# AgoraIO-Community/Solo

Hardware: AMD Instinct MI355X
Metric: 40 ms frames/sec (encode+decode) per GPU; concurrent real-time WB streams @1/2/4/8 MI355X (higher is better)
Workload: dtype int32 fixed point (int16 PCM, Q-format arithmetic, bit-exact); 1 GPU; BASELINE configs[2]: 4096 synthetic 16 kHz WB streams, full encode -> two-description bitstream -...; streams_per_gpu=4096, input_workers=16, launch=single process

## Files before the change

solo_amd/csrc/solo_common.h:

```cpp
#pragma once
#include "solo_wave.h"

#if defined(__HIPCC__)
#define SOLO_TAB static __device__ const
#else
#define SOLO_TAB static const
#endif
#include "solo_tables.inc"

#ifndef SX_FS_KHZ
#define SX_FS_KHZ 8
#endif
#if SX_FS_KHZ == 8
#define SX_LPC 10
#define SX_NLSF_STAGES 6
#define SX_NLSF_CB0_NVEC_TOTAL 120
#define SX_NLSF_CB1_NVEC_TOTAL 72
#define SX_NLSF_CB_MAXVEC 120
#define SX_MSVQ_ROW 16
#define SX_N_NLSF_CB0_CDF 126
#define SX_N_NLSF_CB1_CDF 78
#define SX_N_PITCH_LAG_CDF 130
#define SX_N_PITCH_CONTOUR_CDF 12
#define SX_PITCH_CB_N 11
// ... 356 lines not shown
        const u32 tot = sx_uadd_sat(nrg, pre);
        const unsigned long long cross = __builtin_amdgcn_ballot_w64(tot >= 0x80000000u);
        if (!cross) { nrg = (u32)__builtin_amdgcn_readlane((i32)tot, 63); break; }
        const int Lc = __builtin_ctzll(cross);
        u32 base = nrg;
        if (Lc > 0) base += (u32)__builtin_amdgcn_readlane((i32)pre, Lc - 1);
        bool found = false;
#pragma unroll
        for (int j = 0; j < MAXC; j++) {
            const int m = Lc * C + j;
            const u32 pj = (u32)__builtin_amdgcn_readlane((i32)P[j], Lc);
            if (!found && j < C && m >= cur) {
                base += pj >> shft;
                if (base >= 0x80000000u) { found = true; cur = m + 1; }
            }
        }
        nrg = base >> 2;
        shft += 2;
    }
    if (tail) nrg += (u32)sx_smulbb(x[len - 1], x[len - 1]) >> shft;
    if (nrg & 0xC0000000u) { nrg >>= 2; shft += 2; }
    *shift = shft;
    *energy = (i32)nrg;
}
template <int MAXC = 4>
SX_FN void sx_sum_sqr_shift_wv(i32* energy, i32* shift, const i16* x, int len, int odd_start) { sx_sum_sqr_shift_wv_inl<MAXC>(energy, shift, x, len, odd_start); }
#else
template <int MAXC = 4>
SX_HD void sx_sum_sqr_shift_wv(i32* energy, i32* shift, const i16* x, int len, int odd_start) { sx_sum_sqr_shift(energy, shift, x, len, odd_start); }
template <int MAXC>
SX_HD void sx_sum_sqr_shift_wv_inl(i32* energy, i32* shift, const i16* x, int len, int odd_start) { sx_sum_sqr_shift(energy, shift, x, len, odd_start); }
#endif

SX_HD void sx_lpc_analysis_filter_zero_state(const i16* in, const i16* B, i16* out, int len, int order) {
    SX_PAR(k, len) {
        i32 acc = 0;
        for (int j = 0; j < order; j++) {
            int t = k - 1 - j;
            if (t >= 0) acc = sx_smlabb(acc, in[t], B[j]);
        }
        i32 o = sx_sub_sat32(sx_shl((i32)in[k], 12), acc);
        out[k] = (i16)sx_sat16(sx_rshift_round(o, 12));
    }
}

SX_HD i32 sx_sigm_Q15(i32 in_Q5) {
    if (in_Q5 < 0) {
        in_Q5 = -in_Q5;
        if (in_Q5 >= 6 * 32) return 0;
        int ind = in_Q5 >> 5;
        return T_sigm_neg_Q15[ind] - sx_smulbb(T_sigm_slope_Q10[ind], in_Q5 & 0x1F);
    }
    if (in_Q5 >= 6 * 32) return 32767;
    int ind = in_Q5 >> 5;
    return T_sigm_pos_Q15[ind] + sx_smulbb(T_sigm_slope_Q10[ind], in_Q5 & 0x1F);
}

#ifdef SX_LANE_STREAM
#define SX_ROWB(v, jj) __shfl((v), (SX_LANE & 48) | (jj), 64)
#define SX_ROWG(v, idx) __shfl((v), (SX_LANE & 48) | ((idx) & 15), 64)
#define SX_ROW_NEXT(v) SX_DPP_((v), 0x101)

SX_HD void sx_row_nlsf_weights_laroia(i32* pW_Q6, const i32* pNLSF_Q15, int D, bool row_active) {
    const int k = SX_LANE & 15;
    i32 inv = 0;
    if (row_active && k <= D) {
        const i32 lo = k > 0 ? pNLSF_Q15[k - 1] : 0, hi = k < D ? pNLSF_Q15[k] : (1 << 15);
        inv = (1 << 21) / sx_max(hi - lo, 3);
    }
    const i32 nx = SX_ROW_NEXT(inv);
    if (row_active && k < D) pW_Q6[k] = sx_min(inv + nx, 32767);
}

template <int ORDER>
SX_HD i32 sx_row_inv_pred_gain_Q16_n(i32 a, bool* unstable) {
// ... 86 lines not shown
```

solo_amd/csrc/solo_enc.h:

```cpp
#pragma once
#include <stddef.h>
#include "solo_enc_analysis.h"
#if defined(SOLO_HOST_EMU)
#include "solo_enc_nsq_row.h"
#endif
#include "solo_cdf.h"

struct SxFrameIdx {
    i32 sigtype, QuantOffsetType;
    i32 GainsIndices[SX_NB_SUBFR], DeltaGainsIndices;
    i32 NLSFIndices[SX_NLSF_STAGES], NLSFInterpCoef_Q2;
    i32 lagIndex, contourIndex, PERIndex, LTPIndex[SX_NB_SUBFR], LTP_scaleIndex;
    i32 Seed, vadFlag;
    i32 inDTX, pad_;
};

#define SX_RC_PW_SIGNS (SX_FRAME + 2 * (SX_FRAME / 16) + 8 - ((SX_FRAME + 2 * (SX_FRAME / 16)) & 7))
#define SX_RC_PW_ROW (SX_RC_PW_SIGNS + SX_FRAME / 8 + (((SX_RC_PW_SIGNS + SX_FRAME / 8) / 4) & 1 ? 0 : 4))
static_assert(((SX_RC_PW_ROW / 4) & 1) == 1 && SX_RC_PW_ROW % 4 == 0, "odd dword rows");
#define SX_RC_BUF_STRIDE (SX_MAX_ARITHM_BYTES + 16)
struct SxRcInfo { i32 nBytes, error; };

struct SxCodeWork {
#if SX_NLANES == 1
    u8 buf[2][SX_RC_BUF_STRIDE];
    alignas(4) u8 pulses[SX_RC_PW_ROW];
    SxCdf cdf;
#else
    i32 unused_;
#endif
};

struct SxFrontWork {
    i16 x_buf[SX_XBUF];
    i16 res_pitch[2 * SX_FRAME + SX_LA_PITCH];
    i16 Wsig[SX_PITCH_LPC_WIN];
    union {
        SxPitchWork pitch;
        SxShapeWork shape;
        SxPredWork pred;
        SxPrefWork pref;
    } u;
};

struct SxHbWork {
    i16 x_hb_buf[SX_HB_XBUF];
    i16 lpc_in[4 * (10 * SX_FS_KHZ + SX_HB_LPC)];
    i16 exc[2 * SX_FRAME];
    i32 NLSF_Q15[SX_MAX_LPC];
    i32 weight[SX_MAX_LPC];
    i16 A_Q12[SX_MAX_LPC];
    i32 ws[SX_NLSF2A_WS];
    SxLpcWork lpc;
};

#define SX_HB_Q (SX_FS_KHZ == 8 ? 10 : 8)
struct SxEncWork {
    SxEncState st;
    SxEncCtrl ctrl;
    i16 xfw[SX_FRAME];
    u8 hb_bytes[8 * SX_HB_Q];
    union {
        i16 qmf_tl[63 + SX_PACKET];
        SxFrontWork front;
#if defined(SOLO_HOST_EMU)
        SxRowWork nsq;
#endif
        SxCodeWork code;
        SxHbWork hb;
    } u;
};

SX_HD void sx_enc_split(SxRangeEnc* rc, int p_child1, int p, const u16* shell_table, const SxCdf* cdf) {
    if (p > 0) sx_rc_enc(rc, p_child1, &shell_table[cdf->shell_offsets[p]]);
}

// ... 529 lines not shown
```

solo_amd/csrc/solo_enc_analysis.h:

```cpp
#pragma once
#include "solo_enc_front.h"
#include "solo_dec.h"

SX_FN void sx_warped_autocorr(i32* corr, i32* scale, const i16* input, i32 warping_Q16, int length) {
    const int order = SX_SHAPE_ORDER;
    i32 state[SX_SHAPE_ORDER + 1];
    i64 corr_QC[SX_SHAPE_ORDER + 1];
    for (int i = 0; i <= order; i++) { state[i] = 0; corr_QC[i] = 0; }
    for (int n = 0; n < length; n++) {
        i32 tmp1 = sx_shl((i32)input[n], 14), tmp2;
        for (int i = 0; i < order; i += 2) {
            tmp2 = sx_smlawb(state[i], state[i + 1] - tmp1, warping_Q16);
            state[i] = tmp1;
            corr_QC[i] += sx_smull(tmp1, state[0]) >> 18;
            tmp1 = sx_smlawb(state[i + 1], state[i + 2] - tmp2, warping_Q16);
            state[i + 1] = tmp2;
            corr_QC[i + 1] += sx_smull(tmp2, state[0]) >> 18;
        }
        state[order] = tmp1;
        corr_QC[order] += sx_smull(tmp1, state[0]) >> 18;
    }
    int lsh = sx_clz64(corr_QC[0]) - 35;
    lsh = sx_limit(lsh, -12 - 10, 30 - 10);
    *scale = -(10 + lsh);
// ... 1149 lines not shown
SX_FN void sx_burg_modified(i32* res_nrg, i32* res_nrg_Q, i32* A_Q16, const i16* x, int subfr_length, int nb_subfr, i32 WhiteNoiseFrac_Q32,
                            int D, SxBurgWork* bw) {
    SX_IN_LDS(x); SX_IN_LDS(bw); SX_IN_LDS(A_Q16);
    const int QA = 25, MAX_RSHIFTS = 32 - 25, MIN_RSHIFTS = -16;
    subfr_length = SX_UNI(subfr_length); nb_subfr = SX_UNI(nb_subfr); D = SX_UNI(D); WhiteNoiseFrac_Q32 = SX_UNI(WhiteNoiseFrac_Q32);
    const int L = subfr_length;
    i32 C0, rshifts;
    SX_T_BEGIN
    constexpr int PAIRS_PER_LANE = SITE == 2 ? (4 * (10 * SX_FS_KHZ + SX_HB_LPC) / 2 + 63) / 64 : (4 * (SX_SUBFR + SX_MAX_LPC) / 2 + 63) / 64;
    sx_sum_sqr_shift_wv_inl<PAIRS_PER_LANE>(&C0, &rshifts, x, nb_subfr * subfr_length, 0);
    C0 = SX_UNI(C0); rshifts = SX_UNI(rshifts);
    SX_T(23)
    if (rshifts > MAX_RSHIFTS) {
        C0 = sx_shl(C0, rshifts - MAX_RSHIFTS);
        rshifts = MAX_RSHIFTS;
    } else {
        int lz = sx_clz32(C0) - 1;
        int rshifts_extra = 2 - lz;
        if (rshifts_extra > 0) {
            rshifts_extra = sx_min(rshifts_extra, MAX_RSHIFTS - rshifts);
            C0 = C0 >> rshifts_extra;
        } else {
            rshifts_extra = sx_max(rshifts_extra, MIN_RSHIFTS - rshifts);
            C0 = sx_shl(C0, -rshifts_extra);
        }
        rshifts += rshifts_extra;
    }
    C0 = SX_UNI(C0); rshifts = SX_UNI(rshifts);
#if defined(SX_BURG_COUNT) && SX_NLANES == 1
    SX_BURG_COUNTED(SITE, rshifts > -2 ? 0 : 1);
    if (SITE == 1 && sx_burg_last_regime == (rshifts > 0)) SX_BURG_COUNTED(SITE, 3);
    if (SITE == 0) sx_burg_last_regime = rshifts > 0;
#endif
    SX_PAR(sn, nb_subfr * 16) {
        const int s = sn >> 4, n = (sn & 15) + 1;
        i32 v = 0;
        if (n <= D) {
            const i16* xs = x + s * L;
            if (rshifts > 0) {
                i64 acc = 0;
                for (int i = 0; i < L - n; i++) acc += (i64)((i32)xs[i] * (i32)xs[i + n]);
                v = (i32)(acc >> rshifts);
            } else {
                i32 acc = 0;
                for (int i = 0; i < L - n; i++) acc = sx_smlabb(acc, xs[i], xs[i + n]);
                v = sx_shl(acc, -rshifts);
            }
        }
        bw->p1[sn] = v;
    }
    wv_sync();
    SX_PAR(k, SX_MAX_LPC) {
        i32 v = 0;
        for (int s = 0; s < nb_subfr; s++) v = sx_add(v, bw->p1[s * 16 + k]);
        bw->Cf[k] = v;
        bw->Cl[k] = v;
        bw->Af[k] = 0;
    }
    SX_T(24)
    const i32 CA0 = sx_add(sx_add(C0, sx_smmul(WhiteNoiseFrac_Q32, C0)), 1);
    bw->CAf[0] = CA0;
    bw->CAb[0] = CA0;
    wv_sync();
#if defined(__HIP_DEVICE_COMPILE__) && SX_NLANES == 64 && SX_FS_KHZ == 8
    i32 nrg, tmp1;
    {
        const int row = SX_LANE >> 4, k = SX_LANE & 15, rowbase = SX_LANE & 48;
        const bool live = row < nb_subfr;
        const i16* xr = x + (live ? row : 0) * L;
        const bool upper = row >= 2;
        i32 Af_k = 0, P_k = upper ? (k == 0 ? CA0 : 0) : bw->Cf[k], Q_k = P_k;
        i32 ef = live ? (i32)xr[k] : 0, eb = live ? (i32)xr[L - 1 - k] : 0, fr = 0, bk = 0;
#define SX_ROW_DOWN(v) __builtin_amdgcn_update_dpp(0, (v), 0x101, 0xF, 0xF, true)
#define SX_ROW_UP_IN(in, v) __builtin_amdgcn_update_dpp((in), (v), 0x111, 0xF, 0xF, false)
#define SX_ROW_BCAST0(v) __builtin_amdgcn_update_dpp(0, (v), 0x150, 0xF, 0xF, true)
// ... 426 lines not shown
                    i++;
                    if (i > 30) {
                        NLSF[0] = (1 << 15) / (d + 1);
                        for (k = 1; k < d; k++) NLSF[k] = sx_smulbb(k + 1, NLSF[0]);
                        wv_sync();
                        return;
                    }
                    wv_sync();
                    sx_bwexpander_32(a_Q16, d, 65536 - sx_smulbb(10 + i, i));
                    retry = true;
                    break;
                }
            }
        }
#endif
        wv_sync();
        if (!retry) return;
    }
}

SX_FN1 void sx_find_LPC(i32* NLSF_Q15, i32* interpIndex, const i32* prev_NLSFq_Q15, int useInterp, int order, const i16* x,
                       int subfr_length, i16* LPC_res, SxLpcWork* lw) {
    SX_IN_LDS(NLSF_Q15); SX_IN_LDS(interpIndex); SX_IN_LDS(prev_NLSFq_Q15); SX_IN_LDS(x); SX_IN_LDS(LPC_res); SX_IN_LDS(lw);
    i32* a_Q16 = lw->a_Q16;
    i32* a_tmp_Q16 = lw->a_tmp_Q16;
    i32 res_nrg, res_tmp_nrg, res_nrg_Q, res_tmp_nrg_Q;
    order = SX_LPC; subfr_length = SX_SUBFR + SX_LPC;
    *interpIndex = 4;
    sx_burg_modified(&res_nrg, &res_nrg_Q, a_Q16, x, subfr_length, 4, K_FIND_LPC_COND_FAC_Q32, order, &lw->burg);
    sx_bwexpander_32(a_Q16, order, K_FIND_LPC_CHIRP_Q16);
    wv_sync();
    SX_T_BEGIN
    if (useInterp == 1) {
        sx_burg_modified<1>(&res_tmp_nrg, &res_tmp_nrg_Q, a_tmp_Q16, x + 2 * subfr_length, subfr_length, 2, K_FIND_LPC_COND_FAC_Q32, order, &lw->burg);
        sx_bwexpander_32(a_tmp_Q16, order, K_FIND_LPC_CHIRP_Q16);
        wv_sync();
        SX_T(22)
        int shift = res_tmp_nrg_Q - res_nrg_Q;
        if (shift >= 0) {
            if (shift < 32) res_nrg = res_nrg - (res_tmp_nrg >> shift);
        } else {
            res_nrg = (res_nrg >> (-shift)) - res_tmp_nrg;
            res_nrg_Q = res_tmp_nrg_Q;
        }
        sx_a2nlsf<1>(NLSF_Q15, a_tmp_Q16, order, lw->P, lw->Q, &lw->u.grid);
        wv_sync();
        SX_T(21)
#if defined(SX_LANE_STREAM) && defined(SX_HAVE_ROW_NLSF2A)
        bool all_ok;
        {
            const int k = SX_LANE >> 4, i = SX_LANE & 15;
            if (i < SX_LPC) lw->u.it.NLSF0[k][i] = prev_NLSFq_Q15[i] + (sx_mul(NLSF_Q15[i] - prev_NLSFq_Q15[i], k) >> 2);
            wv_sync();
            all_ok = __builtin_amdgcn_ballot_w64(!sx_row_nlsf2a_stable(lw->u.it.a_Q12[k], lw->u.it.NLSF0[k])) == 0;
            wv_sync();
        }
        if (!all_ok)
#endif
        {
            SX_S(55)
            SX_PAR(k, 4) {
                for (int i = 0; i < order; i++) lw->u.it.NLSF0[k][i] = prev_NLSFq_Q15[i] + (sx_mul(NLSF_Q15[i] - prev_NLSFq_Q15[i], k) >> 2);
                sx_nlsf2a_stable_ws(lw->u.it.a_Q12[k], lw->u.it.NLSF0[k], order, lw->u.it.ws[k]);
            }
            wv_sync();
        }
        SX_S(53)
        {
            const int len = 2 * (SX_SUBFR + SX_LPC);
            SX_PAR(t, 4 * len) {
                const int k = t / len, n = t - k * len;
                const i16* B = lw->u.it.a_Q12[k];
                i32 acc = 0;
                for (int j = 0; j < order; j++) {
                    const int u = n - 1 - j;
                    if (u >= 0) acc = sx_smlabb(acc, x[u], B[j]);
                }
                const i32 o = sx_sub_sat32(sx_shl((i32)x[n], 12), acc);
                lw->u.it.res[k][n] = (i16)sx_sat16(sx_rshift_round(o, 12));
            }
        }
        wv_sync();
        SX_S(54)
        SX_PAR(kh, 8) {
            const int k = kh >> 1, h = kh & 1;
            i32 e, sh;
            sx_sum_sqr_shift_n<SX_SUBFR>(&e, &sh, lw->u.it.res[k] + order + h * subfr_length, 0);
            lw->u.it.nrg[k][h] = e;
            lw->u.it.rsh[k][h] = sh;
        }
        wv_sync();
        for (int k = 3; k >= 0; k--) {
            i32 res_nrg0 = lw->u.it.nrg[k][0], res_nrg1 = lw->u.it.nrg[k][1], res_nrg_interp, res_nrg_interp_Q;
            const i32 rshift0 = lw->u.it.rsh[k][0], rshift1 = lw->u.it.rsh[k][1];
            shift = rshift0 - rshift1;
            if (shift >= 0) {
                res_nrg1 = res_nrg1 >> shift;
                res_nrg_interp_Q = -rshift0;
            } else {
                res_nrg0 = res_nrg0 >> (-shift);
                res_nrg_interp_Q = -rshift1;
            }
            res_nrg_interp = sx_add(res_nrg0, res_nrg1);
            shift = res_nrg_interp_Q - res_nrg_Q;
            int isInterpLower;
            if (shift >= 0) {
                isInterpLower = (res_nrg_interp >> shift) < res_nrg;
            } else {
                isInterpLower = (-shift < 32) ? (res_nrg_interp < (res_nrg >> (-shift))) : 0;
            }
            if (isInterpLower) {
                res_nrg = res_nrg_interp;
// ... 344 lines not shown
    if (doInterpolate) {
        SX_PAR(i, SX_LPC) w->NLSF0[i] = st->prev_NLSFq_Q15[i] + (sx_mul(pNLSF_Q15[i] - st->prev_NLSFq_Q15[i], interp_Q2) >> 2);
        wv_sync();
    }
#if defined(SX_LANE_STREAM) && defined(SX_HAVE_ROW_NLSF2A)
    bool both_ok;
    {
        const int v = (SX_LANE >> 4) & 1;
        bool ok = true;
        if (doInterpolate) ok = sx_row_nlsf2a_stable(c->PredCoef_Q12[v], v ? pNLSF_Q15 : w->NLSF0);
        else ok = sx_row_nlsf2a_stable(c->PredCoef_Q12[1], pNLSF_Q15);
        both_ok = __builtin_amdgcn_ballot_w64(!ok) == 0;
        wv_sync();
    }
    if (!both_ok)
#endif
    {
        SX_S(56)
        SX_PAR(v, 2) {
            if (v == 1 || doInterpolate) sx_nlsf2a_stable_ws(c->PredCoef_Q12[v], v ? pNLSF_Q15 : w->NLSF0, SX_LPC, w->ws[v]);
        }
        wv_sync();
    }
    if (!doInterpolate) {
        SX_PAR(i, SX_LPC) c->PredCoef_Q12[0][i] = c->PredCoef_Q12[1][i];
        wv_sync();
    }
}

SX_FN1 void sx_residual_energy(i32* nrgs, i32* nrgsQ, const i16* x, i16 a_Q12[2][SX_MAX_LPC], const i32* gains, i16* LPC_res) {
    const int offset = SX_LPC + SX_SUBFR;
    const i16* x_ptr = x;
    for (int i = 0; i < 2; i++) {
        sx_lpc_analysis_filter_zero_state(x_ptr, a_Q12[i], LPC_res, 2 * offset, SX_LPC);
        wv_sync();
        for (int j = 0; j < 2; j++) {
            i32 rshift;
            static_assert(SX_SUBFR <= 128, "one pair of samples per lane");
            sx_sum_sqr_shift_wv_inl<1>(&nrgs[i * 2 + j], &rshift, LPC_res + SX_LPC + j * offset, SX_SUBFR, 0);
            nrgsQ[i * 2 + j] = -rshift;
        }
        x_ptr += 2 * offset;
        wv_sync();
    }
    for (int i = 0; i < 4; i++) {
        int lz1 = sx_clz32(nrgs[i]) - 1, lz2 = sx_clz32(gains[i]) - 1;
        i32 tmp32 = sx_shl(gains[i], lz2);
        tmp32 = sx_smmul(tmp32, tmp32);
        nrgs[i] = sx_smmul(tmp32, sx_shl(nrgs[i], lz1));
        nrgsQ[i] += lz1 + 2 * lz2 - 32 - 32;
    }
}

struct SxPredWork {
    i32 WLTP[4 * 25];
    i16 LPC_in_pre[4 * (SX_SUBFR + SX_LPC)];
    i16 LPC_res[2 * (SX_SUBFR + SX_LPC)];
    i32 NLSF_Q15[SX_MAX_LPC];
    i32 invGains_Q16[SX_NB_SUBFR], local_gains[SX_NB_SUBFR], Wght_Q15[SX_NB_SUBFR];
    union {
        SxLtpWork ltp;
        struct { i32 rd[3 * 4 * 40]; i32 best[3 * 4 * 2]; } vq;
        SxLpcWork lpc;
        SxMsvqWork msvq;
    } u;
};

// ... 134 lines not shown
```

solo_amd/csrc/solo_enc_front.h:

```cpp
#pragma once
#include "solo_enc_state.h"

SX_FN1 void sx_qmf_decomp(SxEncHist* hist, const i16* pcm, i16* tl, i16* lo, i16* hi, int n = SX_PACKET) {
    SX_IN_LDS(tl);
    n = SX_UNI(n);
    SX_PAR(i, 63) tl[i] = hist->qmf_hist[i];
    SX_PAR(i, n) tl[63 + i] = (i16)(pcm[i] >> 1);
    wv_sync();
    SX_PAR(k, n >> 1) {
        i32 y1 = 0, y2 = 0;
        const i16* xa = tl + 2 * k;
        const i16* xb = tl + 63 + 2 * k;
        for (int j = 0; j < 32; j++) {
            i32 a = T_qmf_taps[63 - j];
            i32 p = xa[j], q = xb[-j];
            y1 = sx_add(y1, sx_mul(a, (i32)(i16)(p + q)));
            i32 d = sx_mul(a, (i32)(i16)(p - q));
            y2 = (j & 1) ? sx_add(y2, d) : sx_sub(y2, d);
        }
        lo[k] = (i16)sx_saturate(sx_pshr32(y1, 15), 32767);
        hi[k] = (i16)sx_saturate(sx_pshr32(y2, 15), 32767);
    }
    wv_sync();
    SX_PAR(i, 63) hist->qmf_hist[i] = tl[n + i];
// ... 528 lines not shown
    const int min_lag_4 = 8, max_lag_4 = 72, min_lag_8 = 16, max_lag_8 = 144, sf8 = 40;
    constexpr int dn_C = (int)((offsetof(SxPitchWork, C) - offsetof(SxPitchWork, tmp32)) / sizeof(i32));
    static_assert(offsetof(SxPitchWork, tmp32) % 16 == 0 && offsetof(SxPitchWork, C) % 16 == 0 && sizeof(w->tmp32) >= 160 * sizeof(i32) &&
                  sizeof(w->C) >= 160 * sizeof(i32), "all-pass chains of the 8 -> 4 kHz decimator");
#if SX_FS_KHZ == 8
    SX_PAR(i, 320) w->sig8[i] = signal[i];
    wv_sync();
#else
    static_assert(offsetof(SxPitchWork, sig16) + sizeof(w->sig16) - offsetof(SxPitchWork, C) >= 640 * sizeof(i32), "all-pass chains of the 16 -> 8 kHz decimator");
    sx_down2_zero_state<640>(w->sig8, signal, w->tmp32 + dn_C, 320);
#endif
    sx_down2_zero_state<320>(w->sig4, w->sig8, w->tmp32, dn_C);
    SX_PAR(i, 4 * 221) (&w->C[0][0])[i] = 0;
#if SX_NLANES == 1
    for (int i = 159; i > 0; i--) w->sig4[i] = (i16)sx_sat16((i32)w->sig4[i] + (i32)w->sig4[i - 1]);
#else
    {
        i32 a[3];
#pragma unroll
        for (int j = 0; j < 3; j++) {
            const int i = SX_LANE + 64 * j;
            a[j] = (i > 0 && i < 160) ? sx_sat16((i32)w->sig4[i] + (i32)w->sig4[i - 1]) : 0;
        }
        wv_sync();
#pragma unroll
        for (int j = 0; j < 3; j++) { const int i = SX_LANE + 64 * j; if (i > 0 && i < 160) w->sig4[i] = (i16)a[j]; }
        wv_sync();
    }
#endif
    i32 shift = sx_pitch_find_scaling(w->sig4, 160, sx_max(sf8, 80));
    if (shift > 0) {
        SX_PAR(i, 160) w->sig4[i] = (i16)(w->sig4[i] >> shift);
        wv_sync();
    }
    SX_S(34)
    {
        i32 E8k[2], N8k[2];
        for (int k = 0; k < 2; k++) {
            const i16* b = &w->sig4[80 + k * sf8] - min_lag_4;
            i32 E8 = 0;
            SX_PAR(n, sf8) E8 = sx_smlabb(E8, b[n], b[n]);
            E8 = wv_sum(E8);
            E8k[k] = E8;
            N8k[k] = sx_add_sat32(E8, sx_smulbb(sf8, 4000));
        }
        const int nlag = max_lag_4 - min_lag_4 + 1;
        SX_PAR(t, 2 * nlag) {
            const int k = t / nlag, d = min_lag_4 + (t - k * nlag);
            const i16* target = &w->sig4[80 + k * sf8];
            const i16* b = target - d;
            i32 cc = 0, E = 0;
            for (int n = 0; n < sf8; n++) { cc = sx_smlabb(cc, target[n], b[n]); E = sx_smlabb(E, b[n], b[n]); }
            i32 normalizer = sx_add(k ? N8k[1] : N8k[0], sx_sub(E, k ? E8k[1] : E8k[0]));
            i32 tq = cc / (sx_sqrt_approx(normalizer) + 1);
            w->C[k][d] = (i16)sx_sat16(tq);
        }
        wv_sync();
    }
    SX_PAR(i, max_lag_4 + 1) {
        if (i >= min_lag_4) {
            i32 sum = ((i32)w->C[0][i] + (i32)w->C[1][i]) >> 1;
            sum = sx_smlawb(sum, sum, sx_shl(-i, 4));
            w->tmp32[i] = sum;
        }
    }
    wv_sync();
    int length_d_srch = 4 + 2 * 2;
    const int L = max_lag_4 - min_lag_4 + 1;
#if SX_NLANES == 64 && defined(__HIP_DEVICE_COMPILE__)
    {
        static_assert(72 - 8 + 1 == 65, "one element more than lanes");
        const int i = SX_LANE;
        const i32 v = (i16)w->tmp32[min_lag_4 + i], vl = (i16)w->tmp32[min_lag_4 + L - 1];
        int rank = 0;
        for (int j = 0; j < L; j++) {
            i32 u = (i16)w->tmp32[min_lag_4 + j];
            rank += (u > v || (u == v && j < i)) ? 1 : 0;
        }
        const int rank_last = __builtin_popcountll(__builtin_amdgcn_ballot_w64(v >= vl));
        wv_sync();
        if (rank < length_d_srch) { w->C[0][min_lag_4 + rank] = (i16)v; w->d_srch[rank] = i; }
        if (SX_LANE == 0 && rank_last < length_d_srch) { w->C[0][min_lag_4 + rank_last] = (i16)vl; w->d_srch[rank_last] = L - 1; }
    }
#else
    SX_PAR(i, L) {
// ... 64 lines not shown
        for (int j = 0; j < 3; j++) { const int i = SX_LANE + 64 * j; if (i >= min_lag_8 && i <= max_lag_8 + 3) w->d_comp[i] = (i16)m[j]; }
        wv_sync();
        int n_srch = 0;
#pragma unroll
        for (int j = 0; j < 3; j++) {
            const int i = SX_LANE + 64 * j;
            const bool pr = i >= min_lag_8 && i <= max_lag_8 && w->d_comp[i + 1] > 0;
            const unsigned long long bal = __builtin_amdgcn_ballot_w64(pr);
            if (pr) w->d_srch[n_srch + __builtin_popcountll(bal & below)] = i;
            n_srch += __builtin_popcountll(bal);
        }
        length_d_srch = n_srch;
#pragma unroll
        for (int j = 0; j < 3; j++) {
            const int i = SX_LANE + 64 * j;
            m[j] = (i >= min_lag_8 && i <= max_lag_8 + 3) ? (i32)w->d_comp[i] + w->d_comp[i - 1] + w->d_comp[i - 2] + w->d_comp[i - 3] : 0;
        }
        wv_sync();
#pragma unroll
        for (int j = 0; j < 3; j++) {
            const int i = SX_LANE + 64 * j;
            const bool pr = i >= min_lag_8 && i <= max_lag_8 + 3 && m[j] > 0;
            const unsigned long long bal = __builtin_amdgcn_ballot_w64(pr);
            if (pr) w->d_comp[length_d_comp + __builtin_popcountll(bal & below)] = (i16)(i - 2);
            length_d_comp += __builtin_popcountll(bal);
        }
        wv_sync();
    }
#endif
    SX_S(35)
    shift = sx_pitch_find_scaling(w->sig8, 320, sf8);
    if (shift > 0) {
        SX_PAR(i, 320) w->sig8[i] = (i16)(w->sig8[i] >> shift);
    }
    SX_PAR(i, 4 * 221) (&w->C[0][0])[i] = 0;
    wv_sync();
    SX_PAR(t, 4 * length_d_comp) {
        int k = t / length_d_comp, j = t - k * length_d_comp;
        const i16* tp = &w->sig8[160 + k * sf8];
        int d = w->d_comp[j];
        const i16* bp = tp - d;
        i32 cross = 0, eb = 0, et = 0;
        for (int n = 0; n < sf8; n++) {
            cross = sx_smlabb(cross, tp[n], bp[n]);
            eb = sx_smlabb(eb, bp[n], bp[n]);
            et = sx_smlabb(et, tp[n], tp[n]);
        }
        i32 r = 0;
        if (cross > 0) {
            i32 en = sx_max(et, eb);
            i32 lz = sx_clz32(cross);
            i32 lshift = sx_limit(lz - 1, 0, 15);
            i32 t32 = sx_shl(cross, lshift) / ((en >> (15 - lshift)) + 1);
            t32 = sx_smulwb(cross, t32);
            t32 = sx_add_sat32(t32, t32);
            lz = sx_clz32(t32);
            lshift = sx_limit(lz - 1, 0, 15);
            en = sx_min(et, eb);
            r = sx_shl(t32, lshift) / ((en >> (15 - lshift)) + 1);
        }
        w->C[k][d] = (i16)r;
    }
    wv_sync();
    i32 CCmax = SX_I32_MIN, CCmax_b = SX_I32_MIN;
    int CBimax = 0, lag = -1;
#if SX_FS_KHZ == 16
    if (prevLag > 0) prevLag = prevLag >> 1;
#endif
    i32 prevLag_log2_Q7 = prevLag > 0 ? sx_lin2log(prevLag) : 0;
    i32 corr_thres_Q15 = sx_smulbb(search_thres2_Q15, search_thres2_Q15) >> 13;
    SX_S(36)
    const int nb_cbks = SX_FS_KHZ == 8 ? 11 : 3;
#if SX_NLANES == 1
    for (int k = 0; k < length_d_srch; k++) {
        int d = w->d_srch[k];
        i32 CCmax_new = SX_I32_MIN;
        int CBimax_new = 0;
        for (int j = 0; j < nb_cbks; j++) {
            i32 cc = 0;
            for (int i = 0; i < 4; i++) cc += (i32)w->C[i][d + T_pitch_cb_stage2[i * 11 + j]];
// ... 19 lines not shown
    {
        i32 best_b = SX_I32_MIN, best_k = SX_I32_MAX, my_cc = 0, my_cb = 0;
        const int k = SX_LANE;
        if (k < length_d_srch) {
            const int d = w->d_srch[k];
            i32 CCmax_new = SX_I32_MIN;
            int CBimax_new = 0;
            for (int j = 0; j < nb_cbks; j++) {
                i32 cc = 0;
                for (int i = 0; i < 4; i++) cc += (i32)w->C[i][d + T_pitch_cb_stage2[i * 11 + j]];
                if (cc > CCmax_new) { CCmax_new = cc; CBimax_new = j; }
            }
            i32 lag_log2_Q7 = sx_lin2log(d);
            i32 CCmax_new_b = CCmax_new - (sx_smulbb(4 * 6554, lag_log2_Q7) >> 7);
            if (prevLag > 0) {
                i32 dl = lag_log2_Q7 - prevLag_log2_Q7;
                dl = sx_smulbb(dl, dl) >> 7;
                i32 bias = sx_smulbb(4 * 6554, *LTPCorr_Q15) >> 15;
                bias = sx_mul(bias, dl) / (dl + (1 << 6));
                CCmax_new_b -= bias;
            }
            if (CCmax_new_b > SX_I32_MIN && CCmax_new > corr_thres_Q15 && T_pitch_cb_stage2[CBimax_new] <= min_lag_8) {
                best_b = CCmax_new_b; best_k = k; my_cc = CCmax_new; my_cb = CBimax_new;
            }
        }
        wv_argmax(&best_b, &best_k);
        if (best_k != SX_I32_MAX && best_b > SX_I32_MIN) {
            CCmax = wv_bcast(my_cc, best_k);
            CBimax = wv_bcast(my_cb, best_k);
            lag = w->d_srch[best_k];
        }
    }
#endif
    if (lag == -1) {
        for (int k = 0; k < 4; k++) pitch_out[k] = 0;
        *LTPCorr_Q15 = 0; *lagIndex = 0; *contourIndex = 0;
        return 1;
    }
#if SX_FS_KHZ == 8
    CCmax = sx_max(CCmax, 0);
    *LTPCorr_Q15 = sx_sqrt_approx(sx_shl(CCmax, 13));
    for (int k = 0; k < 4; k++) pitch_out[k] = lag + T_pitch_cb_stage2[k * 11 + CBimax];
    *lagIndex = lag - min_lag_8;
    *contourIndex = CBimax;
    return 0;
#else
    const int min_lag = 2 * 16, max_lag = 18 * 16, sf = 80;
    shift = sx_pitch_find_scaling(signal, 640, sf);
    SX_PAR(i, 640) w->sig16[i] = (i16)(shift > 0 ? (signal[i] >> shift) : signal[i]);
    lag = sx_limit(lag << 1, min_lag, max_lag);
    const int start_lag = sx_max(lag - 2, min_lag), end_lag = sx_min(lag + 2, max_lag);
    int lag_new = lag;
    *LTPCorr_Q15 = sx_sqrt_approx(sx_shl(CCmax, 13));
    wv_sync();
    const i16* lr = &T_pitch_lag_range_stage3[2 * 4 * 2];
    SX_PAR(t, 4 * 24) {
        const int k = t / 24, jj = t - k * 24, lo = lr[2 * k], hi = lr[2 * k + 1];
        if (jj <= hi - lo) {
            const i16* tp = &w->sig16[4 * sf + k * sf];
            const i16* bp = tp - (start_lag + lo + jj);
            i32 cc = 0;
            for (int n = 0; n < sf; n++) cc = sx_smlabb(cc, tp[n], bp[n]);
            w->corr3[k][jj] = cc;
        }
    }
    SX_PAR(k, 4) {
// ... 121 lines not shown
            if (j == k) rcv = rc;
            const bool in = j < ORD - k;
            const i32 Dn = in ? sx_smlawb(D, sx_shl(C1, 1), rc) : D;
            if (in) C1 = sx_smlawb(C1, sx_shl(D, 1), rc);
            D = SX_ROW_NEXT(Dn);
        }
        const i32 res_nrg = SX_RDLANE(C1, 0);
        c->predGain_Q16 = sx_div32_varQ(c0, sx_max(res_nrg, 1), 16);
        i32 A = 0;
        sx_row_k2a_steps<0, ORD>(A, rcv, j);
        i32 a = sx_sat16(A >> 12);
        {
            i32 chirp_Q16 = K_FIND_PITCH_BANDWITH_EXPANSION_Q16, mine = chirp_Q16;
            const i32 chirp_minus_one_Q16 = chirp_Q16 - 65536;
            for (int i = 1; i < ORD; i++) {
                chirp_Q16 = sx_add(chirp_Q16, sx_rshift_round(sx_mul(chirp_Q16, chirp_minus_one_Q16), 16));
                if (j == i) mine = chirp_Q16;
            }
            a = (i16)sx_rshift_round(sx_mul(mine, a), 16);
        }
#pragma unroll
        for (int d = 0; d < ORD; d++) A_Q12[d] = (i16)SX_RDLANE(a, d);
        (void)auto_corr; (void)A_Q24; (void)rc_Q15; (void)scale;
    }
#else
    sx_autocorr(auto_corr, &scale, Wsig, SX_PITCH_LPC_WIN, SX_PITCH_LPC_ORDER + 1);
    auto_corr[0] = sx_smlawb(auto_corr[0], auto_corr[0], K_FIND_PITCH_WHITE_NOISE_FRACTION_Q16);
    i32 res_nrg = sx_schur(rc_Q15, auto_corr, SX_PITCH_LPC_ORDER);
    c->predGain_Q16 = sx_div32_varQ(auto_corr[0], sx_max(res_nrg, 1), 16);
    sx_k2a(A_Q24, rc_Q15, SX_PITCH_LPC_ORDER);
    for (int i = 0; i < SX_PITCH_LPC_ORDER; i++) A_Q12[i] = (i16)sx_sat16(A_Q24[i] >> 12);
    sx_bwexpander(A_Q12, SX_PITCH_LPC_ORDER, K_FIND_PITCH_BANDWITH_EXPANSION_Q16);
#endif
    SX_PAR(k, buf_len) {
        i32 acc = 0;
        for (int d = 0; d < SX_PITCH_LPC_ORDER; d++) {
            int t = k - 1 - d;
            if (t >= 0) acc = sx_smlabb(acc, x_buf[t], A_Q12[d]);
        }
        i32 o = sx_rshift_round(sx_sub(sx_shl((i32)x_buf[k], 12), acc), 12);
        res[k] = k < SX_PITCH_LPC_ORDER ? (i16)0 : (i16)sx_sat16(o);
    }
    wv_sync();
    i32 thr = K_0p45_Q15;
    thr = sx_smlabb(thr, K_m0p004_Q15, SX_PITCH_LPC_ORDER);
    thr = sx_smlabb(thr, K_m0p1_Q7, st->speech_activity_Q8);
    thr = sx_smlabb(thr, K_0p15_Q15, st->prev_sigtype);
    thr = sx_smlawb(thr, K_m0p1_Q16, c->input_tilt_Q15);
    thr = sx_sat16(thr);
    SX_S(33)
    c->sigtype = sx_pitch_analysis_core(res, c->pitchL, &c->lagIndex, &c->contourIndex, &st->LTPCorr_Q15, st->prevLag,
                                        K_FIND_PITCH_CORRELATION_THRESHOLD_HC_MODE_Q16, (i16)thr, pw);
}
```

solo_amd/csrc/solo_fix.h:

```cpp
#pragma once
#include <stdint.h>

#if defined(__HIPCC__)
#define SX_HD __host__ __device__ __forceinline__
#define SX_DEV __device__
#if defined(SX_INLINE_ALL)
#define SX_FN __host__ __device__ __forceinline__
#else
#define SX_FN static __host__ __device__ __attribute__((noinline))
#endif
#else
#define SX_HD static inline
#define SX_DEV
#define SX_FN static
#endif
#if defined(__HIPCC__) && defined(SX_INLINE_SINGLE)
#define SX_FN1 __host__ __device__ __forceinline__
#else
#define SX_FN1 SX_FN
#endif
#if defined(__HIPCC__) && !defined(SX_OUTLINE_WRAPPERS)
#define SX_FNW __host__ __device__ __forceinline__
#else
#define SX_FNW SX_FN
// ... 17 lines not shown
typedef int32_t i32;
typedef uint32_t u32;
typedef int16_t i16;
typedef uint16_t u16;
typedef int64_t i64;
typedef uint64_t u64;
typedef uint8_t u8;
typedef int8_t i8;

#define SX_I32_MAX 0x7FFFFFFF
#define SX_I32_MIN ((i32)0x80000000)

SX_HD i32 sx_add(i32 a, i32 b) { return (i32)((u32)a + (u32)b); }
SX_HD i32 sx_sub(i32 a, i32 b) { return (i32)((u32)a - (u32)b); }
SX_HD i32 sx_mul(i32 a, i32 b) { return (i32)((u32)a * (u32)b); }
SX_HD i32 sx_shl(i32 a, int s) { return (i32)((u32)a << s); }
SX_HD i32 sx_neg(i32 a) { return (i32)(0u - (u32)a); }
SX_HD i32 sx_min(i32 a, i32 b) { return a < b ? a : b; }
SX_HD i32 sx_max(i32 a, i32 b) { return a > b ? a : b; }
SX_HD i32 sx_abs(i32 a) { return a > 0 ? a : sx_neg(a); }
SX_HD i32 sx_limit(i32 a, i32 l1, i32 l2) {
    return l1 > l2 ? (a > l1 ? l1 : (a < l2 ? l2 : a)) : (a > l2 ? l2 : (a < l1 ? l1 : a));
}

SX_HD i32 sx_smulwb(i32 a, i32 b) { return (i32)(((i64)a * (i64)(i32)((u32)b << 16)) >> 32); }
SX_HD i32 sx_smlawb(i32 acc, i32 a, i32 b) { return sx_add(acc, sx_smulwb(a, b)); }
SX_HD i32 sx_pre16(i32 b) { return (i32)((u32)b << 16); }
SX_HD i32 sx_smulw_pre(i32 a, i32 bs) { return (i32)(((i64)a * (i64)bs) >> 32); }
SX_HD i32 sx_smlaw_pre(i32 acc, i32 a, i32 bs) { return sx_add(acc, sx_smulw_pre(a, bs)); }
SX_HD i32 sx_smulwt(i32 a, i32 b) { return (i32)(((i64)a * (i64)(i32)((u32)b & 0xFFFF0000u)) >> 32); }
SX_HD i32 sx_smlawt(i32 acc, i32 a, i32 b) { return sx_add(acc, sx_smulwt(a, b)); }
SX_HD i32 sx_smulbb(i32 a, i32 b) { return (i32)(i16)a * (i32)(i16)b; }
SX_HD i32 sx_smlabb(i32 acc, i32 a, i32 b) { return sx_add(acc, sx_smulbb(a, b)); }
SX_HD i32 sx_smulbt(i32 a, i32 b) { return sx_mul((i32)(i16)a, b >> 16); }
SX_HD i32 sx_smultt(i32 a, i32 b) { return sx_mul(a >> 16, b >> 16); }
SX_HD i32 sx_rshift_round(i32 a, int s) { return s == 1 ? sx_add(a >> 1, a & 1) : (sx_add(a >> (s - 1), 1) >> 1); }
SX_HD i32 sx_rshift_round_small(i32 a, int s) { return sx_add(a, 1 << (s - 1)) >> s; }
SX_HD i64 sx_rshift_round64(i64 a, int s) { return s == 1 ? (a >> 1) + (a & 1) : (((a >> (s - 1)) + 1) >> 1); }
SX_HD i32 sx_smulww(i32 a, i32 b) { return (i32)(((i64)a * (i64)b) >> 16); }
SX_HD i32 sx_smlaww(i32 acc, i32 a, i32 b) { return sx_add(acc, sx_smulww(a, b)); }
SX_HD i32 sx_smmul(i32 a, i32 b) { return (i32)(((i64)a * (i64)b) >> 32); }
SX_HD i64 sx_smull(i32 a, i32 b) { return (i64)a * (i64)b; }

SX_HD i32 sx_sat16(i32 a) { return a > 32767 ? 32767 : (a < -32768 ? -32768 : a); }
SX_HD i32 sx_add_sat32(i32 a, i32 b) {
    i64 s = (i64)a + (i64)b;
    return s > SX_I32_MAX ? SX_I32_MAX : (s < (i64)SX_I32_MIN ? SX_I32_MIN : (i32)s);
}
SX_HD i32 sx_sub_sat32(i32 a, i32 b) {
    i64 s = (i64)a - (i64)b;
    return s > SX_I32_MAX ? SX_I32_MAX : (s < (i64)SX_I32_MIN ? SX_I32_MIN : (i32)s);
}
SX_HD i32 sx_add_pos_sat32(i32 a, i32 b) { i32 s = sx_add(a, b); return (s & 0x80000000) ? SX_I32_MAX : s; }
SX_HD i32 sx_lshift_sat32(i32 a, int s) {
    i32 lo = SX_I32_MIN >> s, hi = SX_I32_MAX >> s;
    i32 c = a < lo ? lo : (a > hi ? hi : a);
    return sx_shl(c, s);
}

SX_HD i32 sx_clz32(i32 x) {
#if defined(__HIP_DEVICE_COMPILE__)
    return x == 0 ? 32 : __clz(x);
#else
    return x == 0 ? 32 : __builtin_clz((u32)x);
#endif
}
// ... 113 lines not shown
```

solo_amd/csrc/solo_l0_probe.h:

```cpp
#pragma once
#include "solo_common.h"

SX_HD i32 sx_l0_probe(int op, i32 a, i32 b, i32 c) {
    switch (op) {
        case 0: return sx_smulwb(a, b);
        case 1: return sx_smulwt(a, b);
        case 2: return sx_smulww(a, b);
        case 3: return sx_smlawb(c, a, b);
        case 4: return sx_smmul(a, b);
        case 5: return sx_smulbb(a, b);
        case 6: return sx_smlabb(c, a, b);
        case 7: return sx_smulbt(a, b);
        case 8: return sx_smultt(a, b);
        case 9: return sx_rshift_round(a, b);
        case 10: return sx_sat16(a);
        case 11: return sx_add_sat32(a, b);
        case 12: return sx_sub_sat32(a, b);
        case 13: return sx_add_pos_sat32(a, b);
        case 14: return sx_lshift_sat32(a, b);
        case 15: return sx_clz32(a);
        case 16: return sx_ror32(a, b);
        case 17: return sx_sqrt_approx(a);
        case 18: return sx_lin2log(a);
        case 19: return sx_log2lin(a);
        case 20: return sx_div32_varQ(a, b, c);
        case 21: return sx_inverse32_varQ(a, b);
        case 22: return sx_sigm_Q15(a);
        case 23: return sx_rand(a);
        case 24: return sx_limit(a, b, c);
        case 25: return sx_smlaww(c, a, b);
        case 26: return sx_smlawt(c, a, b);
        case 27: return sx_clz16((i16)a);
        case 28: return sx_abs(a);
        case 30: return sx_smulw_pre(a, sx_pre16(b));
        case 31: return sx_smlaw_pre(c, a, sx_pre16(b));
        case 32: return sx_rand_skip(a, (u32)b & 511u);
        case 34: return sx_rshift_round_small(a, b);
        case 35: return sx_inverse32_varQ_pos(a, b);
        case 33: return sx_div_q29(a);
        case 40: return sx_pshr32(a, b);
        case 41: return sx_saturate(a, b);
        case 42: return sx_smulbb(c, (i32)(i16)((i16)a + (i16)b));
        case 43: return sx_smulbb(c, (i32)(i16)((i16)a - (i16)b));
        case 44: return sx_smulbb(a, b);
        case 45: return sx_smlabb(c, a, b);
    }
    return 0;
}
```

Before: 4.475 million 40ms packets/s (encode+decode).

## Use packed int16 dot2 instructions for LPC FIRs, pitch correlations, and Burg autocorr

Replaces scalar int16 multiply-accumulate loops in several encoder hot spots with dword-packed sample pairs fed to the AMD sdot2 instruction, using alignbit to build odd-offset pairs. The affected loops are the LPC analysis filters, the stage-1 and stage-2 pitch correlations, and the small-shift Burg autocorrelation. The goal is to halve the multiply instruction count and the LDS loads in these inner loops. It relies on dword alignment of the buffers, which static_asserts enforce, and on wraparound sums matching the old saturating adds for bit-exactness. It also adds host-only dot-count instrumentation.

```diff
diff --git a/solo_amd/csrc/solo_common.h b/solo_amd/csrc/solo_common.h
--- a/solo_amd/csrc/solo_common.h
+++ b/solo_amd/csrc/solo_common.h
@@ -412,15 +412,15 @@
 SX_HD void sx_sum_sqr_shift_wv_inl(i32* energy, i32* shift, const i16* x, int len, int odd_start) { sx_sum_sqr_shift(energy, shift, x, len, odd_start); }
 #endif
 
-SX_HD void sx_lpc_analysis_filter_zero_state(const i16* in, const i16* B, i16* out, int len, int order) {
+template <int ORDER>
+SX_HD void sx_lpc_analysis_filter_zero_state(const i16* in, const i16* B, i16* out, int len) {
+    u32 B2[ORDER / 2];
+    sx_fir_pack<ORDER>(B2, B);
     SX_PAR(k, len) {
-        i32 acc = 0;
-        for (int j = 0; j < order; j++) {
-            int t = k - 1 - j;
-            if (t >= 0) acc = sx_smlabb(acc, in[t], B[j]);
-        }
-        i32 o = sx_sub_sat32(sx_shl((i32)in[k], 12), acc);
-        out[k] = (i16)sx_sat16(sx_rshift_round(o, 12));
+        i32 xk;
+        const i32 acc = sx_fir_dot2<ORDER>(in, k, B2, &xk);
+        i32 o = sx_sub_sat32(sx_shl(xk, 12), acc);
+        out[k] = k < ORDER ? (i16)0 : (i16)sx_sat16(sx_rshift_round(o, 12));
     }
 }
 
diff --git a/solo_amd/csrc/solo_enc.h b/solo_amd/csrc/solo_enc.h
--- a/solo_amd/csrc/solo_enc.h
+++ b/solo_amd/csrc/solo_enc.h
@@ -42,6 +42,9 @@
         SxPrefWork pref;
     } u;
 };
+
+static_assert(alignof(SxFrontWork) >= 4 && offsetof(SxFrontWork, x_buf) % 4 == 0 && alignof(SxPredWork) >= 4 && offsetof(SxPredWork, LPC_in_pre) % 4 == 0,
+              "int16 arrays that the packed FIRs read as dwords (sx_fir_dot2)");
 
 struct SxHbWork {
     i16 x_hb_buf[SX_HB_XBUF];
diff --git a/solo_amd/csrc/solo_enc_analysis.h b/solo_amd/csrc/solo_enc_analysis.h
--- a/solo_amd/csrc/solo_enc_analysis.h
+++ b/solo_amd/csrc/solo_enc_analysis.h
@@ -1205,6 +1205,7 @@
     if (SITE == 1 && sx_burg_last_regime == (rshifts > 0)) SX_BURG_COUNTED(SITE, 3);
     if (SITE == 0) sx_burg_last_regime = rshifts > 0;
 #endif
+    const bool dwords = SX_UNI((int)((((u32)(uintptr_t)x >> 1) | (u32)L) & 1u)) == 0;
     SX_PAR(sn, nb_subfr * 16) {
         const int s = sn >> 4, n = (sn & 15) + 1;
         i32 v = 0;
@@ -1214,6 +1215,21 @@
                 i64 acc = 0;
                 for (int i = 0; i < L - n; i++) acc += (i64)((i32)xs[i] * (i32)xs[i + n]);
                 v = (i32)(acc >> rshifts);
+            } else if (dwords) {
+                const sx_u32a *aw = sx_dwords(xs), *bw = sx_dwords(xs) + (n >> 1);
+                const int sh = (n & 1) << 4, P = (L - 1 - n) >> 1;
+                u32 lo = bw[0];
+                i32 acc = 0;
+#if defined(__clang__)
+#pragma unroll 8
+#endif
+                for (int m = 0; m < P; m++) {
+                    const u32 hi = bw[m + 1];
+                    acc = sx_dot2(acc, aw[m], sx_pair(lo, hi, sh));
+                    lo = hi;
+                }
+                acc = sx_dot2(acc, aw[P], sx_pair(lo, 0u, sh));
+                v = sx_shl(acc, -rshifts);
             } else {
                 i32 acc = 0;
                 for (int i = 0; i < L - n; i++) acc = sx_smlabb(acc, xs[i], xs[i + n]);
@@ -1706,6 +1722,7 @@
     wv_sync();
     SX_T_BEGIN
     if (useInterp == 1) {
+        SX_DOT_COUNTED(10);
         sx_burg_modified<1>(&res_tmp_nrg, &res_tmp_nrg_Q, a_tmp_Q16, x + 2 * subfr_length, subfr_length, 2, K_FIND_LPC_COND_FAC_Q32, order, &lw->burg);
         sx_bwexpander_32(a_tmp_Q16, order, K_FIND_LPC_CHIRP_Q16);
         wv_sync();
@@ -1744,14 +1761,12 @@
             const int len = 2 * (SX_SUBFR + SX_LPC);
             SX_PAR(t, 4 * len) {
                 const int k = t / len, n = t - k * len;
-                const i16* B = lw->u.it.a_Q12[k];
-                i32 acc = 0;
-                for (int j = 0; j < order; j++) {
-                    const int u = n - 1 - j;
-                    if (u >= 0) acc = sx_smlabb(acc, x[u], B[j]);
-                }
-                const i32 o = sx_sub_sat32(sx_shl((i32)x[n], 12), acc);
-                lw->u.it.res[k][n] = (i16)sx_sat16(sx_rshift_round(o, 12));
+                u32 B2[SX_LPC / 2];
+                sx_fir_pack<SX_LPC>(B2, lw->u.it.a_Q12[k]);
+                i32 xn;
+                const i32 acc = sx_fir_dot2<SX_LPC>(x, n, B2, &xn);
+                const i32 o = sx_sub_sat32(sx_shl(xn, 12), acc);
+                lw->u.it.res[k][n] = n < SX_LPC ? (i16)0 : (i16)sx_sat16(sx_rshift_round(o, 12));
             }
         }
         wv_sync();
@@ -2162,7 +2177,7 @@
     const int offset = SX_LPC + SX_SUBFR;
     const i16* x_ptr = x;
     for (int i = 0; i < 2; i++) {
-        sx_lpc_analysis_filter_zero_state(x_ptr, a_Q12[i], LPC_res, 2 * offset, SX_LPC);
+        sx_lpc_analysis_filter_zero_state<SX_LPC>(x_ptr, a_Q12[i], LPC_res, 2 * offset);
         wv_sync();
         for (int j = 0; j < 2; j++) {
             i32 rshift;
diff --git a/solo_amd/csrc/solo_enc_front.h b/solo_amd/csrc/solo_enc_front.h
--- a/solo_amd/csrc/solo_enc_front.h
+++ b/solo_amd/csrc/solo_enc_front.h
@@ -584,6 +584,7 @@
     if (shift > 0) {
         SX_PAR(i, 160) w->sig4[i] = (i16)(w->sig4[i] >> shift);
         wv_sync();
+        SX_DOT_COUNTED(6);
     }
     SX_S(34)
     {
@@ -599,10 +600,10 @@
         const int nlag = max_lag_4 - min_lag_4 + 1;
         SX_PAR(t, 2 * nlag) {
             const int k = t / nlag, d = min_lag_4 + (t - k * nlag);
-            const i16* target = &w->sig4[80 + k * sf8];
-            const i16* b = target - d;
-            i32 cc = 0, E = 0;
-            for (int n = 0; n < sf8; n++) { cc = sx_smlabb(cc, target[n], b[n]); E = sx_smlabb(E, b[n], b[n]); }
+            static_assert(offsetof(SxPitchWork, sig4) % 4 == 0 && alignof(SxPitchWork) >= 4 && 80 + 40 - 8 + 41 < 160 && 80 - 72 >= 0, "stage-1 windows read as dwords");
+            i32 cc, E;
+            sx_corr_dot2<40, false>(w->sig4, 80 + k * sf8, 80 + k * sf8 - d, &cc, &E, nullptr);
+            SX_DOT_COUNTED(0 + (d & 1));
             i32 normalizer = sx_add(k ? N8k[1] : N8k[0], sx_sub(E, k ? E8k[1] : E8k[0]));
             i32 tq = cc / (sx_sqrt_approx(normalizer) + 1);
             w->C[k][d] = (i16)sx_sat16(tq);
@@ -733,20 +734,17 @@
     shift = sx_pitch_find_scaling(w->sig8, 320, sf8);
     if (shift > 0) {
         SX_PAR(i, 320) w->sig8[i] = (i16)(w->sig8[i] >> shift);
+        SX_DOT_COUNTED(7);
     }
     SX_PAR(i, 4 * 221) (&w->C[0][0])[i] = 0;
     wv_sync();
     SX_PAR(t, 4 * length_d_comp) {
         int k = t / length_d_comp, j = t - k * length_d_comp;
-        const i16* tp = &w->sig8[160 + k * sf8];
         int d = w->d_comp[j];
-        const i16* bp = tp - d;
-        i32 cross = 0, eb = 0, et = 0;
-        for (int n = 0; n < sf8; n++) {
-            cross = sx_smlabb(cross, tp[n], bp[n]);
-            eb = sx_smlabb(eb, bp[n], bp[n]);
-            et = sx_smlabb(et, tp[n], tp[n]);
-        }
+        static_assert(offsetof(SxPitchWork, sig8) % 4 == 0 && 160 + 3 * 40 - (16 - 2) + 41 < 320 && 160 - (144 + 3 - 2) >= 0, "stage-2 windows read as dwords");
+        i32 cross, eb, et;
+        sx_corr_dot2<40, true>(w->sig8, 160 + k * sf8, 160 + k * sf8 - d, &cross, &eb, &et);
+        SX_DOT_COUNTED(2 + (d & 1));
         i32 r = 0;
         if (cross > 0) {
             i32 en = sx_max(et, eb);
@@ -832,6 +830,7 @@
         }
     }
 #endif
+    if (lag != -1) { SX_DOT_COUNTED(4 + (lag & 1)); }
     if (lag == -1) {
         for (int k = 0; k < 4; k++) pitch_out[k] = 0;
         *LTPCorr_Q15 = 0; *lagIndex = 0; *contourIndex = 0;
@@ -1019,13 +1018,13 @@
     for (int i = 0; i < SX_PITCH_LPC_ORDER; i++) A_Q12[i] = (i16)sx_sat16(A_Q24[i] >> 12);
     sx_bwexpander(A_Q12, SX_PITCH_LPC_ORDER, K_FIND_PITCH_BANDWITH_EXPANSION_Q16);
 #endif
+    static_assert(buf_len % 2 == 0 && buf_len <= SX_XBUF && SX_PITCH_LPC_ORDER % 2 == 0, "x_buf read as dwords");
+    u32 A2[SX_PITCH_LPC_ORDER / 2];
+    sx_fir_pack<SX_PITCH_LPC_ORDER>(A2, A_Q12);
     SX_PAR(k, buf_len) {
-        i32 acc = 0;
-        for (int d = 0; d < SX_PITCH_LPC_ORDER; d++) {
-            int t = k - 1 - d;
-            if (t >= 0) acc = sx_smlabb(acc, x_buf[t], A_Q12[d]);
-        }
-        i32 o = sx_rshift_round(sx_sub(sx_shl((i32)x_buf[k], 12), acc), 12);
+        i32 xk;
+        const i32 acc = sx_fir_dot2<SX_PITCH_LPC_ORDER>(x_buf, k, A2, &xk);
+        i32 o = sx_rshift_round(sx_sub(sx_shl(xk, 12), acc), 12);
         res[k] = k < SX_PITCH_LPC_ORDER ? (i16)0 : (i16)sx_sat16(o);
     }
     wv_sync();
@@ -1038,4 +1037,5 @@
     SX_S(33)
     c->sigtype = sx_pitch_analysis_core(res, c->pitchL, &c->lagIndex, &c->contourIndex, &st->LTPCorr_Q15, st->prevLag,
                                         K_FIND_PITCH_CORRELATION_THRESHOLD_HC_MODE_Q16, (i16)thr, pw);
-}
+    SX_DOT_COUNTED(c->sigtype == 0 ? 8 : 9);
+}
diff --git a/solo_amd/csrc/solo_fix.h b/solo_amd/csrc/solo_fix.h
--- a/solo_amd/csrc/solo_fix.h
+++ b/solo_amd/csrc/solo_fix.h
@@ -73,6 +73,76 @@
 SX_HD i32 sx_smlawt(i32 acc, i32 a, i32 b) { return sx_add(acc, sx_smulwt(a, b)); }
 SX_HD i32 sx_smulbb(i32 a, i32 b) { return (i32)(i16)a * (i32)(i16)b; }
 SX_HD i32 sx_smlabb(i32 acc, i32 a, i32 b) { return sx_add(acc, sx_smulbb(a, b)); }
+SX_HD i32 sx_dot2(i32 acc, u32 a2, u32 b2) {
+#if defined(__HIP_DEVICE_COMPILE__)
+    typedef short sx_v2i16_ __attribute__((ext_vector_type(2)));
+    return __builtin_amdgcn_sdot2(__builtin_bit_cast(sx_v2i16_, a2), __builtin_bit_cast(sx_v2i16_, b2), acc, false);
+#else
+    return (i32)((u32)acc + (u32)((i32)(i16)a2 * (i32)(i16)b2) + (u32)((i32)(i16)(a2 >> 16) * (i32)(i16)(b2 >> 16)));
+#endif
+}
+SX_HD u32 sx_pair(u32 lo, u32 hi, int sh) {
+#if defined(__HIP_DEVICE_COMPILE__)
+    return __builtin_amdgcn_alignbit(hi, lo, (u32)sh);
+#else
+    return (u32)(((((u64)hi) << 32) | (u64)lo) >> (sh & 31));
+#endif
+}
+#if defined(SX_DOT_COUNT) && !defined(__HIPCC__)
+extern "C" { inline long long sx_dot_count[16]; }
+#define SX_DOT_COUNTED(what) (sx_dot_count[what]++)
+#else
+#define SX_DOT_COUNTED(what)
+#endif
+SX_HD u32 sx_pack2(i32 lo, i32 hi) { return ((u32)lo & 0xFFFFu) | ((u32)hi << 16); }
+typedef u32 __attribute__((may_alias)) sx_u32a;
+SX_HD const sx_u32a* sx_dwords(const i16* p) { return (const sx_u32a*)(const void*)p; }
+
+template <int ORDER>
+SX_HD i32 sx_fir_dot2(const i16* in, int k, const u32* cp, i32* in_k) {
+    static_assert(ORDER % 2 == 0, "coefficient pairs");
+    const int s0 = k >= ORDER ? k - ORDER : 0;
+    const sx_u32a* w = sx_dwords(in) + (s0 >> 1);
+    const int sh = (k & 1) << 4;
+    u32 dw[ORDER / 2 + 1];
+#if defined(__clang__)
+#pragma unroll
+#endif
+    for (int q = 0; q <= ORDER / 2; q++) dw[q] = w[q];
+    i32 acc = 0;
+#if defined(__clang__)
+#pragma unroll
+#endif
+    for (int q = 0; q < ORDER / 2; q++) acc = sx_dot2(acc, sx_pair(dw[q], dw[q + 1], sh), cp[q]);
+    *in_k = (i32)(i16)(dw[ORDER / 2] >> sh);
+    return acc;
+}
+template <int ORDER>
+SX_HD void sx_fir_pack(u32* cp, const i16* B) {
+    for (int q = 0; q < ORDER / 2; q++) cp[q] = sx_pack2(B[ORDER - 1 - 2 * q], B[ORDER - 2 - 2 * q]);
+}
+
+template <int N, bool WITH_ET>
+SX_HD void sx_corr_dot2(const i16* sig, int ti, int bi, i32* cc, i32* eb, i32* et) {
+    static_assert(N % 2 == 0, "sample pairs");
+    const sx_u32a *tw = sx_dwords(sig) + (ti >> 1), *bw = sx_dwords(sig) + (bi >> 1);
+    const int sh = (bi & 1) << 4;
+    i32 c_ = 0, b_ = 0, t_ = 0;
+    u32 lo = bw[0];
+#if defined(__clang__)
+#pragma unroll
+#endif
+    for (int n = 0; n < N / 2; n++) {
+        const u32 hi = bw[n + 1], tp = tw[n], bp = sx_pair(lo, hi, sh);
+        c_ = sx_dot2(c_, tp, bp);
+        b_ = sx_dot2(b_, bp, bp);
+        if (WITH_ET) t_ = sx_dot2(t_, tp, tp);
+        lo = hi;
+    }
+    *cc = c_; *eb = b_;
+    if (WITH_ET) *et = t_;
+}
+
 SX_HD i32 sx_smulbt(i32 a, i32 b) { return sx_mul((i32)(i16)a, b >> 16); }
 SX_HD i32 sx_smultt(i32 a, i32 b) { return sx_mul(a >> 16, b >> 16); }
 SX_HD i32 sx_rshift_round(i32 a, int s) { return s == 1 ? sx_add(a >> 1, a & 1) : (sx_add(a >> (s - 1), 1) >> 1); }
diff --git a/solo_amd/csrc/solo_l0_probe.h b/solo_amd/csrc/solo_l0_probe.h
--- a/solo_amd/csrc/solo_l0_probe.h
+++ b/solo_amd/csrc/solo_l0_probe.h
@@ -44,6 +44,8 @@
         case 43: return sx_smulbb(c, (i32)(i16)((i16)a - (i16)b));
         case 44: return sx_smulbb(a, b);
         case 45: return sx_smlabb(c, a, b);
+        case 50: return sx_dot2(c, (u32)a, (u32)b);
+        case 51: return (i32)sx_pair((u32)a, (u32)b, (c & 1) << 4);
     }
     return 0;
 }
```

New measurement: 4.633 million 40ms packets/s (encode+decode) (median of 6 runs). 3.5% higher.
